# arkworks-rs/poly-commit

Hardware: AMD Instinct MI355X
Metric: MSM G1-scalar-pairs/sec inside KZG commit+open (MarlinKZG10<Bls12_381> shape, hiding off), inputs HBM-resident (host-input blocking calls: value_trait_shaped) (higher is better)
Workload: dtype u32 limbs (381-bit Fq / 255-bit Fr modular integer); 1 GPU; MarlinKZG10<bls12_381> commit+open, dense poly deg 2^24 per GPU, true SRS resident, hiding off (BASELINE metric sizes: 2^20 = configs[1], 2^24 = north-star target); curve=bls12_381, log_degree=24, inflight=2, srs_window_table=True, parallelism=1 GPU

## Files before the change

### poly_commit_amd/csrc/ec.hpp

```cpp
#pragma once
#include "fp32.hpp"
#include "fp30.hpp"
#include "fp2.hpp"

namespace pc {

template <class C1> struct G2Of { typedef C1 Base; typedef typename C1::FqP FqP; typedef typename C1::FrP FrP; };
template <class C> struct CoordOf { typedef Fd<typename C::FqP> type; };
template <class C1> struct CoordOf<G2Of<C1>> { typedef Fq2D<typename C1::FqP> type; };
template <class C> struct ScalarCurveOf { typedef C type; static constexpr bool IS_G2 = false; };
template <class C1> struct ScalarCurveOf<G2Of<C1>> { typedef C1 type; static constexpr bool IS_G2 = true; };
#ifndef PC_TE_DERIVED_TD
#define PC_TE_DERIVED_TD 1
#endif
template <class T> struct TeOf { typedef T Curve; typedef typename T::FqP FqP; typedef typename T::FrP FrP; };
template <class T> struct CoordOf<TeOf<T>> { typedef Fd<typename T::FqP> type; };
template <class T> struct ScalarCurveOf<TeOf<T>> { typedef TeOf<T> type; static constexpr bool IS_G2 = false; };
template <class C> struct GroupKind {
  static constexpr bool IS_TE = false, TABLE_FREE = ScalarCurveOf<C>::IS_G2, MANY_MSM = !ScalarCurveOf<C>::IS_G2, TWO_LANE = !ScalarCurveOf<C>::IS_G2;
};
template <class T> struct GroupKind<TeOf<T>> { static constexpr bool IS_TE = true, TABLE_FREE = true, MANY_MSM = true, TWO_LANE = false; };

template <class C>
struct AffD {
// ... 34 lines not shown
    r.Y = M.mul_add_mul(S.sub(r.X), W.neg(), a.y);
    r.ZZ = V; r.ZZZ = W;
    return r;
  }
  PC_HD XyzzD dbl() const {
    if (is_inf() || Y.is_zero()) return infinity();
    XyzzD r;
    Fq U = Y.dbl(), V = U.sqr(), W = U.mul(V), S = X.mul(V);
    Fq xx = X.sqr(), M = xx.dbl().add(xx);
    r.X = M.sqr().sub(S.dbl());
    r.Y = M.mul_add_mul(S.sub(r.X), W.neg(), Y);
    r.ZZ = V.mul(ZZ); r.ZZZ = W.mul(ZZZ);
    return r;
  }
  PC_HD void add_affine(const AffD<C>& a) {
    if (a.is_inf()) return;
    if (is_inf()) { X = a.x; Y = a.y; ZZ = Fq::one(); ZZZ = Fq::one(); return; }
    Fq U2 = a.x.mul(ZZ), S2 = a.y.mul(ZZZ);
    Fq Pp = U2.sub(X), R = S2.sub(Y);
    if (Pp.is_zero()) {
      if (R.is_zero()) *this = dbl_affine(a); else *this = infinity();
      return;
    }
    Fq PP = Pp.sqr(), PPP = Pp.mul(PP), Q = X.mul(PP);
    Fq X3 = R.sqr().sub(PPP).sub(Q.dbl());
    Y = R.mul_add_mul(Q.sub(X3), Y.neg(), PPP);
    X = X3;
    ZZ = ZZ.mul(PP); ZZZ = ZZZ.mul(PPP);
  }
  PC_HD void add_affine_lz(const AffD<C>& a, bool negate) {
    if (a.y.is_zero()) { if (a.x.is_zero()) return; }
    const Fq ay = negate ? a.y.neg_lz_canonical() : a.y;
    if (is_inf()) { X = a.x; Y = ay; ZZ = Fq::one(); ZZZ = Fq::one(); return; }
    Fq U2 = a.x.mul_lz(ZZ), S2 = ay.mul_lz(ZZZ);
    Fq Pp = U2.sub_lz(X), R = S2.sub_lz(Y);
    if (Pp.is_zero_lz()) {
      XyzzD t = canonical();
      AffD<C> b; b.x = a.x; b.y = ay.canon();
      t.add_affine(b);
      *this = t;
      return;
    }
    Fq PP = Pp.sqr_lz(), PPP = Pp.mul_lz(PP), Q = X.mul_lz(PP);
    Fq X3 = R.sqr_lz().sub_lz(PPP).sub_lz(Q.dbl_lz());
    Y = R.mul_add_mul_lz(Q.sub_lz(X3), Y.neg_lz(), PPP);
    X = X3;
    ZZ = ZZ.mul_lz(PP); ZZZ = ZZZ.mul_lz(PPP);
  }
  PC_HD XyzzD canonical() const { XyzzD r; r.X = X.canon1(); r.Y = Y.canon1(); r.ZZ = ZZ.canon1(); r.ZZZ = ZZZ.canon1(); return r; }
  PC_HD void add(const XyzzD& o) {
    if (o.is_inf()) return;
    if (is_inf()) { *this = o; return; }
    Fq U1 = X.mul(o.ZZ), U2 = o.X.mul(ZZ), S1 = Y.mul(o.ZZZ), S2 = o.Y.mul(ZZZ);
    Fq Pp = U2.sub(U1), R = S2.sub(S1);
    if (Pp.is_zero()) {
      if (R.is_zero()) *this = dbl(); else *this = infinity();
      return;
    }
    Fq PP = Pp.sqr(), PPP = Pp.mul(PP), Q = U1.mul(PP);
    Fq X3 = R.sqr().sub(PPP).sub(Q.dbl());
    Y = R.mul_add_mul(Q.sub(X3), S1.neg(), PPP);
    X = X3;
    ZZ = ZZ.mul(o.ZZ).mul(PP); ZZZ = ZZZ.mul(o.ZZZ).mul(PPP);
  }
  PC_HD AffD<C> to_affine() const {
    if (is_inf()) return AffD<C>::infinity();
    Fq t = ZZ.mul(ZZZ).inv();
    AffD<C> a; a.x = X.mul(t.mul(ZZZ)); a.y = Y.mul(t.mul(ZZ)); return a;
  }
};


struct XyzzR30 {
  typedef pc_curve_bls12_381 C;
  typedef Fd<C::FqP> F32;
  typedef Fq30 Fq;
  Fq X, Y, ZZ, ZZZ;

  static PC_HD XyzzR30 infinity() { XyzzR30 r; r.X = Fq::zero(); r.Y = Fq::zero(); r.ZZ = Fq::zero(); r.ZZZ = Fq::zero(); return r; }
  PC_HD bool is_inf() const { return ZZ.is_zero_exact(); }
  PC_HD XyzzD<C> to32() const { XyzzD<C> r; r.X = X.to32(); r.Y = Y.to32(); r.ZZ = ZZ.to32(); r.ZZZ = ZZZ.to32(); return r; }
  static PC_HD XyzzR30 from32(const XyzzD<C>& p) {
    XyzzR30 r; r.X = Fq::from32(p.X); r.Y = Fq::from32(p.Y); r.ZZ = Fq::from32(p.ZZ).reduce(); r.ZZZ = Fq::from32(p.ZZZ).reduce(); return r;
  }
  PC_HD void add_affine(const AffD<C>& a, bool negate) {
    if (a.y.is_zero()) { if (a.x.is_zero()) return; }
    const F32 ay32 = negate ? a.y.neg_lz_canonical() : a.y;
    const Fq ax = Fq::from32(a.x), ay = Fq::from32(ay32);
    if (is_inf()) { X = ax; Y = ay; ZZ = Fq::one(); ZZZ = Fq::one(); return; }
    const Fq U2 = Fq::mul<64, 2>(ax, ZZ), S2 = Fq::mul<64, 2>(ay, ZZZ);
    const Fq Pp = Fq::sub<64>(U2, X), R = Fq::sub<64>(S2, Y);
    if (Pp.is_zero_modp<66>()) {
      if (R.is_zero_modp<66>()) { AffD<C> b; b.x = a.x; b.y = ay32.canon(); *this = from32(XyzzD<C>::dbl_affine(b)); }
      else *this = infinity();
      return;
    }
    const Fq PP = Fq::sqr<66>(Pp);
    const Fq PPP = Fq::mul<66, 8>(Pp, PP), Q = Fq::mul<64, 8>(X, PP);
    const Fq RR = Fq::sqr<66>(R);
    const Fq X3 = Fq::sub_dbl<4>(Fq::sub<2>(RR, PPP), Q);
    const Fq T = Fq::sub<14>(Q, X3), NY = Fq::neg<64>(Y);
    Y = Fq::mul_add_mul<66, 16, 64, 2>(R, T, NY, PPP);
    X = X3;
    ZZ = Fq::mul<2, 8>(ZZ, PP); ZZZ = Fq::mul<2, 2>(ZZZ, PPP);
    static_assert(Fq::mul_out(64 * 2) <= 2 && Fq::mul_out(66 * 66) <= 8 && Fq::mul_out(66 * 8) <= 2 && Fq::mul_out(64 * 8) <= 2, "classes of add_affine");
    static_assert(Fq::mul_out(66 * 16 + 64 * 2) <= 64 && 8 + 2 + 4 <= 64 && Fq::mul_out(2 * 8) <= 2 && Fq::mul_out(2 * 2) <= 2, "the invariant closes");
  }
};


template <class C>
struct HalfPt {
  typedef Fd<typename C::FqP> Fq;
  Fq a, b;
  static PC_HD HalfPt of(const XyzzD<C>& p, bool odd) { HalfPt h; h.a = odd ? p.Y : p.X; h.b = odd ? p.ZZZ : p.ZZ; return h; }
};
template <class Fq>
PC_HD Fq fq_sel(bool c, const Fq& x, const Fq& y) {
  Fq r;
  PC_UNROLL for (int i = 0; i < Fq::N; i++) r.l[i] = c ? x.l[i] : y.l[i];
  return r;
}
template <class C>
struct HalfAdd {
  typedef Fd<typename C::FqP> Fq;
  Fq T1, D, DD, BB, T5, rc1, R6, X3;
  PC_HD bool p1(const HalfPt<C>& p, const HalfPt<C>& o) { T1 = p.a.mul(o.b); const Fq T2 = o.a.mul(p.b); D = T2.sub(T1); return D.is_zero(); }
  PC_HD Fq p2(const HalfPt<C>& p, const HalfPt<C>& o, bool odd) { DD = D.sqr(); BB = p.b.mul(o.b); T5 = D.mul(DD); return fq_sel(odd, DD, T5); }
  PC_HD Fq p3(bool odd, const Fq& recv) {
    rc1 = recv;
    R6 = fq_sel(odd, BB, T1).mul(fq_sel(odd, rc1, DD));
    X3 = rc1.sub(T5).sub(R6.dbl());
    return R6.sub(X3);
  }
  PC_HD void p4(HalfPt<C>& p, bool odd, const Fq& rc2) {
    const Fq R7 = fq_sel(odd, D, BB).mul_add_mul(fq_sel(odd, rc2, DD), fq_sel(odd, T1.neg(), Fq::zero()), fq_sel(odd, rc1, Fq::zero()));
    p.a = fq_sel(odd, R7, X3);
    p.b = fq_sel(odd, R6, R7);
  }
};

template <class C>
struct JacD {
  typedef Fd<typename C::FqP> Fq;
  Fq X, Y, Z;
  static PC_HD JacD infinity() { JacD r; r.X = Fq::one(); r.Y = Fq::one(); r.Z = Fq::zero(); return r; }
  PC_HD bool is_inf() const { return Z.is_zero(); }
  PC_HD JacD dbl() const {
    if (is_inf() || Y.is_zero()) return infinity();
    Fq A = X.sqr(), B = Y.sqr(), Cc = B.sqr();
    Fq t = X.add(B).sqr().sub(A).sub(Cc);
    Fq D = t.dbl(), E = A.dbl().add(A), F = E.sqr();
    JacD r;
    r.X = F.sub(D.dbl());
    r.Z = Y.mul(Z).dbl();
    r.Y = E.mul(D.sub(r.X)).sub(Cc.dbl().dbl().dbl());
    return r;
  }
  PC_HD void add_affine(const AffD<C>& a) {
    if (a.is_inf()) return;
    if (is_inf()) { X = a.x; Y = a.y; Z = Fq::one(); return; }
    Fq Z1Z1 = Z.sqr(), U2 = a.x.mul(Z1Z1), S2 = a.y.mul(Z).mul(Z1Z1);
    Fq H = U2.sub(X), rr = S2.sub(Y);
    if (H.is_zero()) {
      if (rr.is_zero()) *this = dbl(); else *this = infinity();
      return;
// ... 76 lines not shown
```

### poly_commit_amd/csrc/msm.hpp

```cpp
#pragma once
#include <stddef.h>
#include <stdint.h>
#include <algorithm>
#include <stdexcept>
#include <vector>
#include "ec.hpp"
#include "glv.hpp"
#include "host_tail.hpp"

#if defined(__HIP_DEVICE_COMPILE__)
#define PC_ARRIVED(PT, IDX)                                                                                             \
  do {                                                                                                                  \
    constexpr int PC_N_ = sizeof((PT).x.l) / 4;                                                                         \
    for (int pc_i_ = 0; pc_i_ < PC_N_; pc_i_ += 4) asm volatile("" ::"v"((PT).x.l[pc_i_]), "v"((PT).y.l[pc_i_]));     \
    asm volatile("" ::"v"(IDX));                                                                                        \
  } while (0)
#define PC_ARRIVED_WORD(W) asm volatile("" ::"v"(W))
#define PC_ARRIVED_TD(PT)                                                                                               \
  do {                                                                                                                  \
    constexpr int PC_N_ = sizeof((PT).td.l) / 4;                                                                        \
    for (int pc_i_ = 0; pc_i_ < PC_N_; pc_i_ += 4) asm volatile("" ::"v"((PT).td.l[pc_i_]));                          \
  } while (0)
#define PC_ARRIVED_FQ2(PT, IDX)                                                                                         \
  do {                                                                                                                  \
// ... 146 lines not shown
    PC_UNROLL for (int h = 0; h < 2; h++) {
      PC_UNROLL for (int k = 0; k < 4; k++) o[5 * h + k] = hv.m[h][k];
      o[5 * h + 4] = hv.m[h][4] | (hv.neg[h] << 31);
    }
  }
};
template <class C, class Geo, class F>
PC_HD void for_each_signed_digit(const Geo& g, const uint32_t* scalar, F f) {
  if constexpr (HasGlv<C>::value) { if (g.glv) { for_each_signed_digit_t<C, 1>(g, scalar, f); return; } }
  for_each_signed_digit_t<C, 0>(g, scalar, f);
}

template <class C>
struct DigitsHistBody {
  typedef typename C::FrP FrP;
  MsmGeom g;
  const uint32_t* scalars;
  uint32_t* hist;
  PC_HD void operator()(uint32_t i) const {
    uint32_t sub, j; g.split(i, sub, j);
    for_each_signed_digit<C>(g, g.scalar_at(scalars, i, sub, j, FrP::N), [&](uint32_t h, uint32_t w, uint32_t mag, uint32_t) {
      atomic_inc_u32(hist + (size_t)g.key_window(w, sub, h) * g.nb_win + (mag - 1));
    });
  }
};

template <class C>
struct ScatterBody {
  typedef typename C::FrP FrP;
  MsmGeom g;
  const uint32_t* scalars;
  uint32_t* cursor;
  uint32_t* entries;
  PC_HD void operator()(uint32_t i) const {
    uint32_t sub, j; g.split(i, sub, j);
    for_each_signed_digit<C>(g, g.scalar_at(scalars, i, sub, j, FrP::N), [&](uint32_t h, uint32_t w, uint32_t mag, uint32_t neg) {
      const uint32_t pos = atomic_inc_u32(cursor + (size_t)g.key_window(w, sub, h) * g.nb_win + (mag - 1));
      entries[pos] = g.base_index(w, j) | (neg << 31);
    });
  }
};

PC_HD uint32_t find_bucket(const uint32_t* offs, uint32_t nb, uint32_t v) {
  uint32_t lo = 0, hi = nb;
  while (hi - lo > 1) {
    uint32_t mid = (lo + hi) >> 1;
    if (offs[mid] <= v) lo = mid; else hi = mid;
  }
  return lo;
}

PC_HD void partial_slot_range(const uint32_t* offs, uint32_t key, uint32_t T, uint32_t T2, uint32_t T2b, uint32_t level,
                              uint32_t& lo, uint32_t& hi) {
  lo = 2 * (offs[key] / T);
  hi = 2 * ((offs[key + 1] - 1) / T);
  for (uint32_t l = 2; l <= level; l++) { const uint32_t d = (l == 2) ? T2 : T2b; lo = 2 * (lo / d); hi = 2 * (hi / d); }
}

template <class C> struct AccSum { static constexpr bool R30 = false; typedef XyzzD<C> type; };
#if PC_ACC_R30
template <> struct AccSum<pc_curve_bls12_381> { static constexpr bool R30 = true; typedef XyzzR30 type; };
#endif
PC_HD constexpr uint32_t acc_stage_word(uint32_t tid, uint32_t piece, uint32_t pieces) { return ((tid >> 6) * pieces + piece) * 256u + (tid & 63u) * 4u; }
template <class C>
struct StageRegs {
  AffD<C> nxt;
  PC_HD void gather(const uint32_t* src) { nxt = AffD<C>::load(src); }
  PC_HD AffD<C> take() const { return nxt; }
  PC_HD void done() const {}
};
template <class C>
struct AccumulateBody {
  typedef XyzzD<C> Pt;
  typedef typename AccSum<C>::type Sum;
  static constexpr bool R30 = AccSum<C>::R30;
  static constexpr int AW = AffD<C>::WORDS;
  MsmGeom g;
  const uint32_t* bases;
  const uint32_t* entries;
  const uint32_t* offsets;
  uint32_t* buckets;
  uint32_t* pkeys;
  uint32_t* ppts;
  static constexpr bool LAZY = Pt::Fq::LAZY_OK;
  static constexpr bool LAZY_STORE = LAZY && Pt::Fq::LAZY_STORE_OK;
  static PC_HD Pt store_form(const Pt& acc) { if constexpr (LAZY && !LAZY_STORE) return acc.canonical(); else return acc; }
  static PC_HD Pt store_form(const XyzzR30& acc) { static_assert(!R30 || LAZY_STORE, "to32() hands over lazily reduced coordinates"); return acc.to32(); }
  PC_HD void flush(const Pt& acc_lz, uint32_t k, bool complete, uint32_t t, bool first, uint32_t& k0, uint32_t& k1) const {
    const Pt& acc = acc_lz;
    if (complete) { acc.store(buckets + (size_t)k * Pt::WORDS); return; }
    uint32_t slot = first ? 2 * t : 2 * t + 1;
    acc.store(ppts + (size_t)slot * Pt::WORDS);
    if (first) k0 = k; else k1 = k;
  }
  template <class Stage = StageRegs<C>>
  PC_HD void chunk(uint32_t t, uint32_t& k0, uint32_t& k1, Pt& last, Stage st = Stage()) const {
    const uint32_t M = offsets[g.NB];
    const uint64_t s64 = (uint64_t)t * g.T;
    k0 = KEY_INVALID; k1 = KEY_INVALID;
    if (s64 < M) {
      const uint32_t s = (uint32_t)s64;
      const uint32_t e = (M - s > g.T) ? s + g.T : M;
      uint32_t k = find_bucket(offsets, g.NB, s);
      uint32_t run_lo = offsets[k], boundary = offsets[k + 1];
      uint32_t next_boundary = offsets[k + 2 <= g.NB ? k + 2 : g.NB];
      Sum acc = Sum::infinity();
      bool first = true;
      uint32_t val = entries[s];
      uint32_t nval = (s + 1 < e) ? entries[s + 1] : val;
      constexpr bool PREFETCH_PT = !ScalarCurveOf<C>::IS_G2;
      AffD<C> pt = AffD<C>::load(bases + (size_t)(val & PC_ACC_DEBUG_IDX_MASK) * g.pt_stride);
      for (uint32_t p = s; p < e; p++) {
        if constexpr (ScalarCurveOf<C>::IS_G2) PC_ARRIVED_FQ2(pt, nval); else PC_ARRIVED(pt, nval);
#if PC_TE_DERIVED_TD
        if constexpr (GroupKind<C>::IS_TE) PC_ARRIVED_TD(pt);
#endif
        PC_ARRIVED_WORD(next_boundary);
        if (p == boundary) {
          flush(store_form(acc), k, run_lo >= s, t, first, k0, k1);
          first = false; acc = Sum::infinity();
          k++; run_lo = p; boundary = next_boundary;
          while (boundary <= p) { k++; boundary = offsets[k + 1]; }
        }
        if constexpr (PREFETCH_PT) {
        st.gather(bases + (size_t)(nval & PC_ACC_DEBUG_IDX_MASK) * g.pt_stride);
        const uint32_t nnval = entries[p + 2 < e ? p + 2 : e - 1];
        next_boundary = offsets[k + 2 <= g.NB ? k + 2 : g.NB];
        if constexpr (R30) acc.add_affine(pt, (val >> 31) != 0);
        else if constexpr (LAZY) acc.add_affine_lz(pt, (val >> 31) != 0); else acc.add_affine(pt.neg_if(val >> 31));
        val = nval; nval = nnval; pt = st.take();
        } else {
          const uint32_t nnval = entries[p + 2 < e ? p + 2 : e - 1];
          next_boundary = offsets[k + 2 <= g.NB ? k + 2 : g.NB];
          acc.add_affine(pt.neg_if(val >> 31));
          val = nval; nval = nnval;
          pt = AffD<C>::load(bases + (size_t)(val & PC_ACC_DEBUG_IDX_MASK) * g.pt_stride);
        }
      }
      st.done();
      if constexpr (R30) {
        last = store_form(acc);
        flush(last, k, run_lo >= s && boundary <= e, t, first, k0, k1);
      } else {
        acc = store_form(acc);
        flush(acc, k, run_lo >= s && boundary <= e, t, first, k0, k1);
        last = acc;
      }
    }
  }
  PC_HD void operator()(uint32_t t) const {
    uint32_t k0, k1; Pt last;
    chunk(t, k0, k1, last);
    pkeys[2 * t] = k0; pkeys[2 * t + 1] = k1;
  }
};

template <class C>
struct SegReduceBody {
  static constexpr bool LATENCY_BOUND = true;
  typedef XyzzD<C> Pt;
  MsmGeom g;
  uint32_t level;
  uint32_t n_in;
  const uint32_t* in_keys; const uint32_t* in_pts;
  const uint32_t* offsets;
  uint32_t* buckets;
  uint32_t* out_keys; uint32_t* out_pts;
  PC_HD void flush(const Pt& acc, uint32_t key, uint32_t cs, uint32_t ce, uint32_t u, bool first, uint32_t& k0, uint32_t& k1) const {
    uint32_t lo, hi; partial_slot_range(offsets, key, g.T, g.T2, g.T2b, level, lo, hi);
    if (lo >= cs && hi < ce) { acc.store(buckets + (size_t)key * Pt::WORDS); return; }
    uint32_t slot = first ? 2 * u : 2 * u + 1;
    acc.store(out_pts + (size_t)slot * Pt::WORDS);
    if (first) k0 = key; else k1 = key;
  }
  PC_HD void operator()(uint32_t u) const {
    const uint32_t T2l = level == 1 ? g.T2 : g.T2b;
    const uint32_t cs = u * T2l;
    const uint32_t ce = (n_in - cs > T2l) ? cs + T2l : n_in;
    uint32_t k0 = KEY_INVALID, k1 = KEY_INVALID;
    uint32_t cur = KEY_INVALID; bool first = true;
    Pt acc = Pt::infinity();
    for (uint32_t p = cs; p < ce; p++) {
      uint32_t key = in_keys[p];
      if (key == KEY_INVALID) continue;
      if (key != cur) {
        if (cur != KEY_INVALID) { flush(acc, cur, cs, ce, u, first, k0, k1); first = false; }
        cur = key; acc = Pt::infinity();
      }
      acc.add(Pt::load(in_pts + (size_t)p * Pt::WORDS));
    }
    if (cur != KEY_INVALID) flush(acc, cur, cs, ce, u, first, k0, k1);
    out_keys[2 * u] = k0; out_keys[2 * u + 1] = k1;
  }
};

template <class C>
struct BucketLevelBody {
  static constexpr bool LATENCY_BOUND = true;
  typedef XyzzD<C> Pt;
  uint32_t K, weight_off, cnt, n_old;
  const uint32_t* x;
  const uint32_t* old_in;
  uint32_t* out;
  PC_HD void operator()(uint32_t lane) const {
    const uint32_t a = lane / cnt, gidx = lane % cnt;
    const size_t stride = (size_t)cnt * Pt::WORDS;
    if (a == 0) {
      const uint32_t* base = x + (size_t)gidx * K * Pt::WORDS;
      Pt run = Pt::infinity(), acc = Pt::infinity();
      if constexpr (ScalarCurveOf<C>::IS_G2) {
        for (uint32_t j = K; j-- > 0;) {
          run.add(Pt::load(base + (size_t)j * Pt::WORDS));
          if (j + weight_off > 0) acc.add(run);
        }
      } else {
      Pt nxt = Pt::load(base + (size_t)(K - 1) * Pt::WORDS);
      for (uint32_t j = K; j-- > 0;) {
        const Pt cur = nxt;
        nxt = Pt::load(base + (size_t)(j > 0 ? j - 1 : 0) * Pt::WORDS);
        run.add(cur);
        if (j + weight_off > 0) acc.add(run);
      }
      }
      run.store(out + (size_t)gidx * Pt::WORDS);
      acc.store(out + stride + (size_t)gidx * Pt::WORDS);
    } else {
      const uint32_t* base = old_in + (size_t)(a - 1) * cnt * K * Pt::WORDS + (size_t)gidx * K * Pt::WORDS;
      Pt acc = Pt::infinity();
      if constexpr (ScalarCurveOf<C>::IS_G2) {
        for (uint32_t j = 0; j < K; j++) acc.add(Pt::load(base + (size_t)j * Pt::WORDS));
      } else {
      Pt nxt = Pt::load(base);
      for (uint32_t j = 0; j < K; j++) {
        const Pt cur = nxt;
        nxt = Pt::load(base + (size_t)(j + 1 < K ? j + 1 : j) * Pt::WORDS);
        acc.add(cur);
// ... 273 lines not shown
inline MsmLevels msm_plan_levels(const MsmConfig& cfg, const MsmGeom& g, size_t n, bool tbl) {
  MsmLevels lv;
  uint32_t m = g.nb_win;
  uint32_t kbits = 0;
  while (m > 1) {
    uint32_t K;
    const size_t level_pts = (size_t)n * g.Wd <= cfg.coop2_max_entries ? (size_t)g.W * m * (1 + (lv.n_levels ? lv.narr[lv.n_levels - 1] : 0))
                                                                         : (size_t)-1;
    if ((size_t)g.W * m > cfg.coop_max_points) K = tbl ? cfg.tbl_K0 : cfg.K0;
    else {
      uint32_t rem = 0; while ((1u << rem) < m) rem++;
      uint32_t lg1 = 0; while ((1u << lg1) < cfg.K1) lg1++;
      if (level_pts <= cfg.coop2_max_points && lg1 > 7) lg1 = 7;
      const uint32_t nl = (rem + lg1 - 1) / lg1;
      K = 1u << ((rem + nl - 1) / nl);
    }
    if (K > m) K = m;
    uint32_t lgK = 0; while ((1u << lgK) < K) lgK++;
    const bool bits = K >= 16;
    const uint32_t woff = lv.n_levels == 0 ? 1u : 0u;
    const uint32_t nw = bits ? lgK + woff : 1u;
    lv.K[lv.n_levels] = K; m /= K; lv.m[lv.n_levels] = m;
    lv.mode[lv.n_levels] = !bits ? 0u : (K <= 128 && level_pts <= cfg.coop2_max_points) ? 2u : 1u;
    lv.narr[lv.n_levels] = nw + (lv.n_levels ? lv.narr[lv.n_levels - 1] : 0);
    std::vector<uint32_t> e;
    if (bits) { for (uint32_t b = 0; b < lgK; b++) e.push_back(kbits + b); if (woff) e.push_back(kbits); }
    else e.push_back(kbits);
    e.insert(e.end(), lv.arr_exp.begin(), lv.arr_exp.end());
    lv.arr_exp.swap(e);
    kbits += lgK;
    lv.n_levels++;
  }
  return lv;
}

template <class C, class Backend>
class MsmPlan {
 public:
  typedef XyzzD<C> Pt;
  typedef typename C::FrP FrP;
  typedef typename ScalarCurveOf<C>::type SC;
  static constexpr bool G2 = GroupKind<C>::TABLE_FREE;
  static constexpr int AW = AffD<C>::WORDS;

  MsmPlan(Backend& be, size_t n_max, const MsmConfig& cfg, uint32_t subs = 0) : be_(be), cfg_(cfg), n_max_(n_max), subs_(subs) {
    if (subs_ && (!cfg_.tbl || !cfg_.tbl_c || n_max % subs_)) throw std::runtime_error("MsmPlan: many-MSM mode needs a window table");
    if (G2 && (subs_ ? !GroupKind<C>::MANY_MSM : cfg_.tbl != nullptr)) throw std::runtime_error("MsmPlan: G2 and twisted Edwards groups are table-free");
    if (cfg_.T2 < 4) cfg_.T2 = 4;
    if (cfg_.T2b < 4) cfg_.T2b = 4;
    auto pow2_floor = [](uint32_t v, uint32_t lo, uint32_t hi) { uint32_t p = lo; while (p * 2 <= v && p * 2 <= hi) p *= 2; return p; };
    cfg_.K0 = pow2_floor(cfg_.K0, 2, 1u << 12);
    cfg_.tbl_K0 = pow2_floor(cfg_.tbl_K0, 2, 1u << 12);
    cfg_.K1 = pow2_floor(cfg_.K1, 2, 256);
    if (cfg_.T2 > 4096) cfg_.T2 = 4096;
    if (cfg_.T2b > 4096) cfg_.T2b = 4096;
    min_T_ = cfg_.T ? cfg_.T : 16;
    size_t NBmax = 1, Mmax = 1, red_max = 1, res_max = 1;
    std::vector<size_t> sizes;
    if (subs_) sizes.push_back(n_max);
    else {
      for (size_t p2 = 1; p2 <= n_max; p2 <<= 1) { sizes.push_back(p2); if (p2 > 1) sizes.push_back(p2 - 1); if (p2 > (n_max >> 1)) break; }
      sizes.push_back(31); sizes.push_back(32); sizes.push_back(n_max);
      if (cfg_.tbl && cfg_.tbl_min_n) { sizes.push_back(cfg_.tbl_min_n); if (cfg_.tbl_min_n > 1) sizes.push_back(cfg_.tbl_min_n - 1); }
    }
    for (size_t n : sizes) {
      if (n < 1 || n > n_max) continue;
      plan_geometry(n);
      NBmax = std::max<size_t>(NBmax, g_.NB);
      Mmax = std::max<size_t>(Mmax, n * (size_t)g_.Wd);
      size_t total = 0;
      for (uint32_t l = 0; l < n_levels_; l++) total += (size_t)(1 + lvl_narr_[l]) * g_.W * lvl_m_[l];
      red_max = std::max(red_max, total);
      res_max = std::max<size_t>(res_max, (size_t)g_.W * (n_levels_ ? lvl_narr_[n_levels_ - 1] : 1));
    }
    entries_cap_ = Mmax; nb_cap_ = NBmax;
    if (!cfg_.T && Mmax <= ((size_t)1 << 17)) min_T_ = 8;
    hist_ = offsets_ = cursor_ = entries_ = buckets_ = scalars_ = red_ = nullptr; pk_[0] = pk_[1] = pp_[0] = pp_[1] = nullptr;
    try {
    hist_ = (uint32_t*)be_.alloc((NBmax + 1) * 4);
    offsets_ = (uint32_t*)be_.alloc((NBmax + 1) * 4);
    cursor_ = (uint32_t*)be_.alloc((NBmax + 1) * 4);
    entries_ = (uint32_t*)be_.alloc(Mmax * 4);
    buckets_ = (uint32_t*)be_.alloc(NBmax * Pt::WORDS * 4);
    scalars_ = (uint32_t*)be_.alloc((n_max ? n_max : 1) * (size_t)FrP::N * 4);
    size_t lanes0 = ceil_div_u32(Mmax, min_T_);
    if (!cfg_.T) {
      const size_t tl = std::max(cfg_.target_lanes, cfg_.tbl ? (cfg_.tbl_chunk ? std::max(cfg_.tbl_max_lanes, cfg_.tbl_target_lanes) : cfg_.tbl_target_lanes) : 0u);
      size_t bound = std::max<size_t>(tl * 17 / 16 + 2, Mmax / 4096 + 1);
      if (lanes0 > bound) lanes0 = bound;
    }
    size_t slots = 2 * lanes0;
    part_slots_ = slots;
    for (int i = 0; i < 2; i++) {
      pk_[i] = (uint32_t*)be_.alloc(slots * 4);
      pp_[i] = (uint32_t*)be_.alloc(slots * (size_t)Pt::WORDS * 4);
      slots = 2 * (size_t)ceil_div_u32(slots, cfg_.T2);
    }
    red_ = (uint32_t*)be_.alloc((red_max + 2 * (size_t)subs_) * (size_t)Pt::WORDS * 4);
    result_host_ = (uint32_t*)be_.alloc_host(std::max<size_t>(res_max, 2 * (size_t)subs_) * Pt::WORDS * 4);
    red_points_ = red_max;
    } catch (...) { release(); throw; }
    plan_geometry(n_max);
  }
  ~MsmPlan() { release(); }
  void release() {
    void* ps[] = {hist_, offsets_, cursor_, entries_, buckets_, scalars_, pk_[0], pk_[1], pp_[0], pp_[1], red_, entries2_, offsets2_, buckets2_, hist2_, cursor2_};
    entries2_ = offsets2_ = buckets2_ = hist2_ = cursor2_ = nullptr;
    for (void* p : ps) be_.free(p);
    be_.free_host(result_host_);
    be_.free(tab_); be_.free_host(tab_host_); tab_ = nullptr; tab_host_ = nullptr;
    hist_ = offsets_ = cursor_ = entries_ = buckets_ = scalars_ = red_ = nullptr; pk_[0] = pk_[1] = pp_[0] = pp_[1] = nullptr;
    result_host_ = nullptr;
  }

  void trim() {
    if (in_parts_) return;
    void* ps[] = {entries2_, offsets2_, buckets2_, hist2_, cursor2_};
    entries2_ = offsets2_ = buckets2_ = hist2_ = cursor2_ = nullptr;
    for (void* p : ps) be_.free(p);
  }

  const MsmGeom& geom() const { return g_; }
  uint32_t* scalar_staging() { return scalars_; }
  const MsmGeom& last_geom() const { return g_; }

  void run(const uint32_t* bases_dev, uint32_t base_off, const uint32_t* scalars_dev, size_t n, bool from_mont,
           uint32_t* out_host) {
    enqueue(bases_dev, base_off, scalars_dev, n, from_mont);
    finish(out_host);
  }

  void enqueue_vectors(const uint32_t* bases_dev, uint32_t base_off, const uint64_t* ptrs_host, size_t count, size_t m, bool from_mont) {
    if (!subs_ || count > subs_ || count * m > n_max_) throw MsmCapacityError("MsmPlan: batch exceeds the plan");
    if (!tab_) { tab_ = (uint64_t*)be_.alloc((size_t)subs_ * 8); tab_host_ = (uint64_t*)be_.alloc_host((size_t)subs_ * 8); }
    for (size_t k = 0; k < count; k++) tab_host_[k] = ptrs_host[k];
    be_.copy_h2d(tab_, tab_host_, count * 8);
    enqueue(bases_dev, base_off, nullptr, count * m, from_mont, m, tab_);
  }

  void enqueue(const uint32_t* bases_dev, uint32_t base_off, const uint32_t* scalars_dev, size_t n, bool from_mont,
               size_t m_sub = 0, const uint64_t* scalar_tab = nullptr) {
    pending_empty_ = (n == 0);
    if (n == 0) return;
    plan_geometry(n);
    parts_k_ = 0; in_parts_ = false;
    part_body(bases_dev, base_off, scalars_dev, n, from_mont, m_sub, scalar_tab, true, true);
    reduce_and_download();
  }

  void begin_parts(size_t n_total) {
    if (subs_) throw std::runtime_error("MsmPlan: parts are for single MSMs");
    pending_empty_ = (n_total == 0);
    if (n_total == 0) return;
    if (n_total > n_max_) throw MsmCapacityError("MsmPlan: call exceeds the workspace this plan was sized for");
    plan_geometry(n_total);
    parts_k_ = 0; in_parts_ = true; parts_n_ = 0;
    if (!entries2_) {
      entries2_ = (uint32_t*)be_.alloc(entries_cap_ * 4);
      offsets2_ = (uint32_t*)be_.alloc((nb_cap_ + 1) * 4);
      buckets2_ = (uint32_t*)be_.alloc(nb_cap_ * Pt::WORDS * 4);
      hist2_ = (uint32_t*)be_.alloc((nb_cap_ + 1) * 4);
      cursor2_ = (uint32_t*)be_.alloc((nb_cap_ + 1) * 4);
    }
    set_tok_[0] = set_tok_[1] = -1;
  }
  void add_part(const uint32_t* bases_dev, uint32_t base_off, const uint32_t* scalars_dev, size_t n, bool from_mont, int ready_tok, bool last) {
    if (pending_empty_ || n == 0) { if (last && !pending_empty_) { if (parts_k_ == 0) { pending_empty_ = true; return; } reduce_and_download(); } return; }
    part_body(bases_dev, base_off, scalars_dev, n, from_mont, 0, nullptr, parts_k_ == 0, last, ready_tok);
    parts_n_ += n;
    if (last) reduce_and_download();
  }

 private:
  void part_body(const uint32_t* bases_dev, uint32_t base_off, const uint32_t* scalars_dev, size_t n, bool from_mont, size_t m_sub,
                 const uint64_t* scalar_tab, bool first, bool last, int ready_tok = -1) {
    MsmGeom g = g_;
    g.n = (uint32_t)n; g.base_off = base_off; g.from_mont = from_mont ? 1 : 0;
    g.m_sub = subs_ ? (uint32_t)(m_sub ? m_sub : n / subs_) : 0u;
    g.scalar_tab = scalar_tab;
    const size_t Mmax = n * g.Wd;
    uint32_t want_lanes = g.tbl_stride ? cfg_.tbl_target_lanes : cfg_.target_lanes;
    if (g.tbl_stride && cfg_.tbl_chunk)
      while ((uint64_t)want_lanes * 2 <= cfg_.tbl_max_lanes && Mmax / ((size_t)want_lanes * 2) >= cfg_.tbl_chunk) want_lanes *= 2;
    uint32_t T = cfg_.T ? cfg_.T : (uint32_t)((Mmax + want_lanes - 1) / want_lanes);
    if (T < min_T_) T = min_T_;
    if (T > 4096) T = 4096;
    g.T = T; g.T2 = cfg_.T2; g.T2b = cfg_.T2b;
    const size_t lanes = ceil_div_u32(Mmax, T);
    if (n > n_max_ || Mmax > entries_cap_ || g.NB > nb_cap_ || 2 * lanes > part_slots_)
      throw MsmCapacityError("MsmPlan: call exceeds the workspace this plan was sized for");
    const int set = in_parts_ ? (int)(parts_k_ & 1u) : 0;
    uint32_t* entries = set ? entries2_ : entries_; uint32_t* offsets = set ? offsets2_ : offsets_;
    uint32_t* hist = set ? hist2_ : hist_; uint32_t* cursor = set ? cursor2_ : cursor_;
    uint32_t* buckets = (in_parts_ && !first) ? buckets2_ : buckets_;
    const bool marks = !in_parts_ || first;
    be_.memset(buckets, 0, (size_t)g.NB * Pt::WORDS * 4);
    if (in_parts_) {
      int tok = -1;
      {
        struct AuxScope { Backend& b; bool marks_was; int* tok; ~AuxScope() { b.timing_marks(marks_was); try { *tok = b.aux_end(); } catch (...) { *tok = -1; } } };
        be_.aux_begin(set_tok_[set], ready_tok);
        AuxScope scope{be_, be_.timing_marks(marks), &tok};
        be_.template sort_entries<SC>(g, scalars_dev, hist, offsets, cursor, entries);
      }
      be_.wait_token(tok);
    } else {
      be_.template sort_entries<SC>(g, scalars_dev, hist, offsets, cursor, entries);
    }

    { AccumulateBody<C> b{g, g.tbl_stride ? cfg_.tbl : bases_dev, entries, offsets, buckets, pk_[0], pp_[0]}; be_.template accumulate<C>(b, lanes); }
    if (!in_parts_ || last) be_.mark();
    const bool tail_queue = !in_parts_ && n <= ((size_t)3 << 19);
    struct TailGuard { Backend& b; bool armed; ~TailGuard() { if (armed) b.end_tail(); } } tail_guard{be_, false};
    if (tail_queue) { be_.begin_tail(); tail_guard.armed = true; }
    size_t slots = 2 * lanes; uint32_t level = 1; int cur = 0;
    for (;;) {
      size_t lanes2 = ceil_div_u32(slots, level == 1 ? g.T2 : g.T2b);
      if (lanes2 <= (cfg_.seg_tail_lanes ? cfg_.seg_tail_lanes : 1u)) {
        be_.template seg_reduce_tail<C>(g, level, (uint32_t)slots, pk_, pp_, cur, offsets, buckets);
        break;
      }
      SegReduceBody<C> b{g, level, (uint32_t)slots, pk_[cur], pp_[cur], offsets, buckets, pk_[cur ^ 1], pp_[cur ^ 1]};
      be_.launch(b, lanes2);
      slots = 2 * lanes2; level++; cur ^= 1;
    }
    if (in_parts_) {
      if (!first) { BucketMergeBody<C> m{buckets_, buckets2_}; be_.launch(m, g.NB); }
      set_tok_[set] = be_.main_token();
      parts_k_++;
    }
    last_g_ = g;
    tail_open_ = tail_queue; tail_guard.armed = false;
  }

  void reduce_and_download() {
    const MsmGeom& g = last_g_;
    struct TailScope { Backend& b; bool on; ~TailScope() { if (on) b.end_tail(); } } tail_scope{be_, tail_open_};
    tail_open_ = false;
    be_.mark();
    const uint32_t* x = buckets_;
    uint32_t* lvl_base = red_;
    uint32_t* prev_base = nullptr;
    for (uint32_t l = 0; l < n_levels_; l++) {
      const uint32_t K = lvl_K_[l], m_out = lvl_m_[l];
      const size_t cnt = (size_t)g.W * m_out;
      const size_t stride = cnt * Pt::WORDS;
      const uint32_t n_old = l ? lvl_narr_[l - 1] : 0;
      const uint32_t* old_in = l ? prev_base + (size_t)g.W * lvl_m_[l - 1] * Pt::WORDS : nullptr;
      be_.template bucket_level<C>(K, l == 0 ? 1u : 0u, (uint32_t)cnt, n_old, (int)lvl_bits_[l], x, old_in, lvl_base);
      x = lvl_base; prev_base = lvl_base; lvl_base += (size_t)(1 + lvl_narr_[l]) * stride;
    }
    be_.mark();
    if (subs_) {
      SubFoldBody<C> f;
      f.arrays = n_levels_ ? prev_base + (size_t)g.W * Pt::WORDS : buckets_;
      f.W = g.W; f.narr = n_levels_ ? (uint32_t)arr_exp_.size() : 1u;
      if (f.narr > 32) throw std::runtime_error("MsmPlan: too many reduction arrays");
      for (uint32_t a = 0; a < f.narr; a++) { f.exp[a] = n_levels_ ? arr_exp_[a] : 0u; f.order[a] = a; }
      std::stable_sort(f.order, f.order + f.narr, [&](uint32_t x, uint32_t y) { return f.exp[x] > f.exp[y]; });
      f.out = red_ + red_points_ * Pt::WORDS;
      be_.launch(f, g.W);
      be_.copy_d2h_async(result_host_, f.out, (size_t)g.W * Pt::WORDS * 4);
    }
    else if (n_levels_ == 0) be_.copy_d2h_async(result_host_, buckets_, (size_t)g.W * Pt::WORDS * 4);
    else be_.copy_d2h_async(result_host_, prev_base + (size_t)g.W * Pt::WORDS, (size_t)g.W * lvl_narr_[n_levels_ - 1] * Pt::WORDS * 4);
    be_.record_done();
    in_parts_ = false;
  }

 public:
  void prepare_replay(size_t n) { pending_empty_ = (n == 0); if (n) plan_geometry(n); }

  void finish(uint32_t* out_host) {
    if (subs_) {
      if constexpr (GroupKind<C>::IS_TE) {
        if (pending_empty_) { std::vector<uint32_t> empty((size_t)subs_ * Pt::WORDS, 0u); host64::batch_to_affine<C>(empty.data(), subs_, out_host); return; }
        be_.wait_done();
        host64::batch_to_affine<C>(result_host_, subs_, out_host);
        return;
      }
      if (pending_empty_) { for (size_t i = 0; i < (size_t)subs_ * AW; i++) out_host[i] = 0; return; }
      be_.wait_done();
      if constexpr (!G2) if (g_.glv) {
        typedef host64::Xyzz64<C> P64;
        std::vector<uint32_t> sum((size_t)subs_ * Pt::WORDS);
        for (uint32_t k = 0; k < subs_; k++) {
          P64 a = P64::load(result_host_ + (size_t)(2 * k) * Pt::WORDS), b = P64::load(result_host_ + (size_t)(2 * k + 1) * Pt::WORDS);
          b.X = b.X.mul(P64::Fq::load(GlvOf<C>::T::BETA_MONT));
          a.add(b);
          a.store(&sum[(size_t)k * Pt::WORDS]);
        }
        host64::batch_to_affine<C>(sum.data(), subs_, out_host);
        return;
      }
      host64::batch_to_affine<C>(result_host_, subs_, out_host);
      return;
    }
    if (pending_empty_) { for (int i = 0; i < AW; i++) out_host[i] = 0; return; }
    if (in_parts_) {
      be_.quiesce();
      in_parts_ = false; tail_open_ = false;
      throw std::runtime_error("MsmPlan: a call in parts was abandoned before its last part");
    }
    be_.wait_done();
    host_tail(out_host);
  }

 private:
  void plan_geometry(size_t n) {
    const bool tbl = subs_ || (cfg_.tbl && cfg_.tbl_c && n >= cfg_.tbl_min_n);
    uint32_t c = tbl ? cfg_.tbl_c : cfg_.c ? cfg_.c : msm_choose_c(n, FrP::BITS);
    g_ = msm_make_geom(FrP::BITS, n, c, tbl, tbl && cfg_.tbl_glv, subs_, cfg_.tbl_stride, tbl ? cfg_.tbl_pt_stride : (uint32_t)AW, cfg_.T2, cfg_.T2b);
    const MsmLevels lv = msm_plan_levels(cfg_, g_, n, tbl);
    n_levels_ = lv.n_levels;
    for (uint32_t l = 0; l < lv.n_levels; l++) { lvl_K_[l] = lv.K[l]; lvl_m_[l] = lv.m[l]; lvl_bits_[l] = lv.mode[l]; lvl_narr_[l] = lv.narr[l]; }
    arr_exp_ = lv.arr_exp;
  }

  void host_tail(uint32_t* out_host) {
    const uint32_t L = n_levels_, W = g_.W;
    const uint32_t cw = g_.tbl_stride ? 0u : g_.c;
    const size_t narr = L == 0 ? 1 : arr_exp_.size();
    if constexpr (!G2) if (g_.glv) {
      typedef host64::Xyzz64<C> P64;
      for (size_t a = 0; a < narr; a++) {
        uint32_t* p = &result_host_[(a * W + 1) * Pt::WORDS];
        P64::Fq::load(p).mul(P64::Fq::load(GlvOf<C>::T::BETA_MONT)).store(p);
      }
    }
    std::vector<host64::WeightedPoint> items;
    if (L == 0) {
      for (uint32_t w = 0; w < W; w++) items.push_back({cw * w, &result_host_[(size_t)w * Pt::WORDS]});
    } else {
      for (size_t a = 0; a < arr_exp_.size(); a++)
        for (uint32_t w = 0; w < W; w++)
          items.push_back({cw * w + arr_exp_[a], &result_host_[(a * W + w) * Pt::WORDS]});
    }
    host64::horner_to_affine<C>(items, out_host);
  }

  Backend& be_;
  MsmConfig cfg_;
  size_t n_max_;
  uint32_t subs_ = 0;
  size_t red_points_ = 0;
  MsmGeom g_;
  uint32_t min_T_;
  size_t part_slots_ = 0, entries_cap_ = 0, nb_cap_ = 0;
  uint32_t *hist_, *offsets_, *cursor_, *entries_, *buckets_, *scalars_, *red_;
  uint32_t* pk_[2]; uint32_t* pp_[2];
  uint32_t n_levels_; uint32_t lvl_K_[32]; uint32_t lvl_m_[32]; uint32_t lvl_bits_[32]; uint32_t lvl_narr_[32];
  std::vector<uint32_t> arr_exp_;
  uint32_t* result_host_ = nullptr;
  uint64_t* tab_ = nullptr; uint64_t* tab_host_ = nullptr;
  bool pending_empty_ = true;
  uint32_t *entries2_ = nullptr, *offsets2_ = nullptr, *buckets2_ = nullptr, *hist2_ = nullptr, *cursor2_ = nullptr;
  uint32_t parts_k_ = 0; size_t parts_n_ = 0; bool in_parts_ = false, tail_open_ = false;
  int set_tok_[2] = {-1, -1};
  MsmGeom last_g_;
};

}
```

### poly_commit_amd/csrc/msm_coop.hpp

```cpp
#pragma once
#include <hip/hip_runtime.h>
#include "msm.hpp"

namespace pc {

template <class C>
struct LdsPoints {
  typedef XyzzD<C> Pt;
  uint32_t* base; uint32_t lanes;
  __device__ __forceinline__ void put(uint32_t lane, const Pt& p) const {
    uint32_t w[Pt::WORDS]; p.store(w);
#pragma unroll
    for (int k = 0; k < Pt::WORDS; k++) base[k * lanes + lane] = w[k];
  }
  __device__ __forceinline__ Pt get(uint32_t lane) const {
    uint32_t w[Pt::WORDS];
#pragma unroll
    for (int k = 0; k < Pt::WORDS; k++) w[k] = base[k * lanes + lane];
    return Pt::load(w);
  }
};

template <class C>
__global__ void __launch_bounds__(256) k_bucket_level_coop(uint32_t K, uint32_t lgK, uint32_t weight_off, uint32_t cnt, uint32_t n_old,
// ... 79 lines not shown
    for (int k = 0; k < FN; k++) { smem[k * L + tid] = v.a.l[k]; smem[(FN + k) * L + tid] = v.b.l[k]; }
  };
  auto get = [&](uint32_t t2) {
    HalfPt<C> r;
#pragma unroll
    for (int k = 0; k < FN; k++) { r.a.l[k] = smem[k * L + t2]; r.b.l[k] = smem[(FN + k) * L + t2]; }
    return r;
  };
  auto store = [&](uint32_t* dst) { v.a.store(dst + oa); v.b.store(dst + ob); };
  if (a == 0) {
    for (uint32_t d = 0; d < lgK; d++) {
      put();
      __syncthreads();
      const uint32_t low = l & ((2u << d) - 1u);
      if ((low & (low - 1u)) == 0 && low < (1u << d)) half_add<C>(v, get(tid + (2u << d)), odd);
      __syncthreads();
    }
    uint32_t* o = out + (size_t)gidx * Pt::WORDS;
    if (l == 0) { store(o); if (weight_off) store(o + (size_t)(1 + lgK) * stride); }
    else if ((l & (l - 1u)) == 0) { uint32_t b = 31 - __builtin_clz(l); store(o + (size_t)(1 + b) * stride); }
  } else {
    for (uint32_t d = K >> 1; d >= 1; d >>= 1) {
      put();
      __syncthreads();
      if (l < d) half_add<C>(v, get(tid + 2 * d), odd);
      __syncthreads();
    }
    if (l == 0) store(out + (size_t)(nw + a) * stride + (size_t)gidx * Pt::WORDS);
  }
}

#ifndef PC_ACC_WAVES_PER_EU
#define PC_ACC_WAVES_PER_EU 1
#endif
#ifndef PC_ACC_WAVES_N8
#define PC_ACC_WAVES_N8 1
#endif
#ifndef PC_ACC_LDS_STAGE
#define PC_ACC_LDS_STAGE 1
#endif
template <class C> struct AccStage { static constexpr bool LDS = PC_ACC_LDS_STAGE && AccSum<C>::R30 && !ScalarCurveOf<C>::IS_G2; };
template <class C>
struct StageLds {
  typedef __attribute__((address_space(3))) uint32_t lds_u32;
  typedef uint32_t u32x4 __attribute__((ext_vector_type(4)));
  typedef __attribute__((address_space(3))) u32x4 lds_u128;
  static constexpr uint32_t PIECES = AffD<C>::WORDS / 4;
  lds_u32* tile; uint32_t tid;
  __device__ __forceinline__ void gather(const uint32_t* src) const {
    const uint32_t wave = __builtin_amdgcn_readfirstlane(tid >> 6);
#pragma unroll
    for (uint32_t j = 0; j < PIECES; j++)
      __builtin_amdgcn_global_load_lds((const __attribute__((address_space(1))) void*)(src + 4 * j),
                                       (__attribute__((address_space(3))) void*)(tile + acc_stage_word(wave << 6, j, PIECES)), 16, 0, 0);
  }
  __device__ __forceinline__ AffD<C> take() const {
    uint32_t w[AffD<C>::WORDS];
#pragma unroll
    for (uint32_t j = 0; j < PIECES; j++) {
      const u32x4 v = *(const lds_u128*)(tile + acc_stage_word(tid, j, PIECES));
      w[4 * j] = v.x; w[4 * j + 1] = v.y; w[4 * j + 2] = v.z; w[4 * j + 3] = v.w;
    }
    return AffD<C>::load(w);
  }
  __device__ __forceinline__ void done() const { asm volatile("s_waitcnt vmcnt(0)" ::: "memory"); }
};
template <class C> struct AccTune {
  static constexpr int WAVES = Fd<typename C::FqP>::N <= 8 ? PC_ACC_WAVES_N8 : (AccSum<C>::R30 && PC_ACC_WAVES_PER_EU < 2) ? 2 : PC_ACC_WAVES_PER_EU;
  static constexpr uint32_t WG = ScalarCurveOf<C>::IS_G2 ? 128u : 256u;
};
#define PC_ACC_BOUNDS __launch_bounds__(AccTune<C>::WG, AccTune<C>::WAVES)
template <class C>
__global__ void PC_ACC_BOUNDS k_accumulate(AccumulateBody<C> b, uint32_t lanes) {
  typedef XyzzD<C> Pt;
  constexpr uint32_t WG = AccTune<C>::WG;
  __shared__ __attribute__((aligned(AccStage<C>::LDS ? 16 : 4))) uint32_t xch[Pt::WORDS * WG];
  __shared__ uint32_t key_out[WG], key_first[WG], flags[WG];
  const uint32_t tid = threadIdx.x, t = blockIdx.x * WG + tid;
  const bool valid = t < lanes;
  uint32_t k0 = KEY_INVALID, k1 = KEY_INVALID;
  Pt V = Pt::infinity();
  if constexpr (AccStage<C>::LDS) {
    static_assert(AffD<C>::WORDS * WG <= Pt::WORDS * WG && WG % 64 == 0, "the stage lies inside the exchange tile");
    if (valid) b.chunk(t, k0, k1, V, StageLds<C>{(typename StageLds<C>::lds_u32*)xch, tid});
  } else {
  if (valid) b.chunk(t, k0, k1, V);
  }
  const uint32_t M = b.offsets[b.g.NB];
  const uint64_t s64 = (uint64_t)t * b.g.T;
  const uint32_t cs = s64 < M ? (uint32_t)s64 : M;
  const uint32_t ce = (M - cs > b.g.T) ? cs + b.g.T : M;
  const bool head_left = k0 != KEY_INVALID && b.offsets[k0] < cs;
  const bool head_right = k0 != KEY_INVALID && k1 == KEY_INVALID && b.offsets[k0 + 1] > ce;
  const bool transparent = head_left && head_right;
  const uint32_t okey = k1 != KEY_INVALID ? k1 : head_right ? k0 : KEY_INVALID;
  LdsPoints<C> lds{xch, WG};
  uint32_t fl = (okey == KEY_INVALID || !transparent) ? 1u : 0u;
  for (uint32_t d = 1; d < WG; d <<= 1) {
    const bool need = !(fl & 1u);
    if (!__syncthreads_or(need)) break;
    if (okey != KEY_INVALID) lds.put(tid, V);
    flags[tid] = fl;
    __syncthreads();
    if (need) {
      if (tid < d) fl = 3u;
      else { V.add(lds.get(tid - d)); fl = flags[tid - d]; }
    }
    __syncthreads();
  }
  key_out[tid] = okey; key_first[tid] = head_left ? k0 : KEY_INVALID; flags[tid] = fl;
  if (okey != KEY_INVALID) lds.put(tid, V);
  __syncthreads();
  const bool take = head_left && tid > 0 && key_out[tid - 1] == k0;
  const bool give = okey != KEY_INVALID && tid < WG - 1 && key_first[tid + 1] == okey;
  if (transparent) {
    if (give) k0 = KEY_INVALID;
    else V.store(b.ppts + (size_t)(2 * t) * Pt::WORDS);
  } else {
    if (take) {
      uint32_t* slot = b.ppts + (size_t)(2 * t) * Pt::WORDS;
      Pt f = Pt::load(slot);
      f.add(lds.get(tid - 1));
      if (!(flags[tid - 1] & 2u) && !head_right) { f.store(b.buckets + (size_t)k0 * Pt::WORDS); k0 = KEY_INVALID; }
      else f.store(slot);
    }
    if (give) { if (k1 != KEY_INVALID) k1 = KEY_INVALID; else k0 = KEY_INVALID; }
  }
  if (valid) { b.pkeys[2 * t] = k0; b.pkeys[2 * t + 1] = k1; }
}

static constexpr uint32_t EDGE_REACH = 8;
template <class C>
__global__ void __launch_bounds__(64) k_accumulate_edges(AccumulateBody<C> b, uint32_t lanes) {
  PC_LATENCY_KERNEL();
  typedef XyzzD<C> Pt;
  constexpr uint32_t WG = AccTune<C>::WG;
  const uint32_t k = blockIdx.x * 64 + threadIdx.x;
  const uint64_t t64 = (uint64_t)(k + 1) * WG;
  if (t64 >= lanes) return;
  const uint32_t t = (uint32_t)t64, a = t - 1;
  const uint32_t M = b.offsets[b.g.NB];
  uint32_t aslot = 2 * a + 1, key = b.pkeys[aslot];
  if (key == KEY_INVALID) {
    aslot = 2 * a; key = b.pkeys[aslot];
    if (key == KEY_INVALID || (uint64_t)b.offsets[key + 1] <= t64 * b.g.T) return;
  }
  uint32_t u = t;
  for (;; u++) {
    if (u >= lanes || u - t >= EDGE_REACH) return;
    const uint32_t ku = b.pkeys[2 * u];
    if (ku == key) break;
    if (ku != KEY_INVALID) return;
  }
  const uint64_t us = (uint64_t)u * b.g.T;
  const uint32_t ue = (M - (uint32_t)us > b.g.T) ? (uint32_t)us + b.g.T : M;
  uint32_t* slot = b.ppts + (size_t)(2 * u) * Pt::WORDS;
  Pt f = Pt::load(slot);
  f.add(Pt::load(b.ppts + (size_t)aslot * Pt::WORDS));
  b.pkeys[aslot] = KEY_INVALID;
  const uint64_t ws = (uint64_t)(a - (WG - 1u)) * b.g.T;
  if (b.offsets[key] >= ws && b.offsets[key + 1] <= ue) { f.store(b.buckets + (size_t)key * Pt::WORDS); b.pkeys[2 * u] = KEY_INVALID; }
  else f.store(slot);
}

template <class C>
__global__ void __launch_bounds__(256) k_seg_reduce_tail(MsmGeom g, uint32_t level, uint32_t slots, uint32_t* pk0, uint32_t* pk1,
                                                         uint32_t* pp0, uint32_t* pp1, int cur, const uint32_t* offsets,
                                                         uint32_t* buckets) {
  PC_LATENCY_KERNEL();
// ... 15 lines not shown
```

Measured before the change: 545.9 million pairs/s.

## Store radix-2^30 bucket sums raw and convert to 32-bit form in a separate pass

Within the accumulate loop, bucket flushes now write the radix-2^30 XYZZ accumulator in its raw limb layout with 128-bit vector stores, skipping the per-flush to32 conversion. Complete buckets go to a new raw buffer and are converted by a follow-up kernel over all buckets. The lane's first partial run is converted in place after the loop. The intent is to take the conversion arithmetic and its register pressure out of the hot accumulation loop. The cost is an extra kernel launch, an extra buffer, and more memory traffic. The LDS-stage path forces RAW=true, which relies on the static_assert that the sum is R30.

```diff
diff --git a/poly_commit_amd/csrc/ec.hpp b/poly_commit_amd/csrc/ec.hpp
--- a/poly_commit_amd/csrc/ec.hpp
+++ b/poly_commit_amd/csrc/ec.hpp
@@ -140,6 +140,29 @@
   PC_HD XyzzD<C> to32() const { XyzzD<C> r; r.X = X.to32(); r.Y = Y.to32(); r.ZZ = ZZ.to32(); r.ZZZ = ZZZ.to32(); return r; }
   static PC_HD XyzzR30 from32(const XyzzD<C>& p) {
     XyzzR30 r; r.X = Fq::from32(p.X); r.Y = Fq::from32(p.Y); r.ZZ = Fq::from32(p.ZZ).reduce(); r.ZZZ = Fq::from32(p.ZZZ).reduce(); return r;
+  }
+  static constexpr int RAW_WORDS = 4 * Fq::N;
+  PC_HD void store_raw(uint32_t* o) const {
+    uint32_t w[RAW_WORDS];
+    PC_UNROLL for (int i = 0; i < Fq::N; i++) { w[i] = X.l[i]; w[Fq::N + i] = Y.l[i]; w[2 * Fq::N + i] = ZZ.l[i]; w[3 * Fq::N + i] = ZZZ.l[i]; }
+#if defined(__HIP_DEVICE_COMPILE__)
+    typedef uint32_t u32x4 __attribute__((ext_vector_type(4)));
+    PC_UNROLL for (int j = 0; j < RAW_WORDS / 4; j++) { u32x4 v; v.x = w[4 * j]; v.y = w[4 * j + 1]; v.z = w[4 * j + 2]; v.w = w[4 * j + 3]; ((u32x4*)o)[j] = v; }
+#else
+    for (int i = 0; i < RAW_WORDS; i++) o[i] = w[i];
+#endif
+  }
+  static PC_HD XyzzR30 load_raw(const uint32_t* p) {
+    uint32_t w[RAW_WORDS];
+#if defined(__HIP_DEVICE_COMPILE__)
+    typedef uint32_t u32x4 __attribute__((ext_vector_type(4)));
+    PC_UNROLL for (int j = 0; j < RAW_WORDS / 4; j++) { const u32x4 v = ((const u32x4*)p)[j]; w[4 * j] = v.x; w[4 * j + 1] = v.y; w[4 * j + 2] = v.z; w[4 * j + 3] = v.w; }
+#else
+    for (int i = 0; i < RAW_WORDS; i++) w[i] = p[i];
+#endif
+    XyzzR30 r;
+    PC_UNROLL for (int i = 0; i < Fq::N; i++) { r.X.l[i] = w[i]; r.Y.l[i] = w[Fq::N + i]; r.ZZ.l[i] = w[2 * Fq::N + i]; r.ZZZ.l[i] = w[3 * Fq::N + i]; }
+    return r;
   }
   PC_HD void add_affine(const AffD<C>& a, bool negate) {
     if (a.y.is_zero()) { if (a.x.is_zero()) return; }
diff --git a/poly_commit_amd/csrc/msm.hpp b/poly_commit_amd/csrc/msm.hpp
--- a/poly_commit_amd/csrc/msm.hpp
+++ b/poly_commit_amd/csrc/msm.hpp
@@ -252,6 +252,7 @@
   uint32_t* buckets;
   uint32_t* pkeys;
   uint32_t* ppts;
+  uint32_t* buckets_raw;
   static constexpr bool LAZY = Pt::Fq::LAZY_OK;
   static constexpr bool LAZY_STORE = LAZY && Pt::Fq::LAZY_STORE_OK;
   static PC_HD Pt store_form(const Pt& acc) { if constexpr (LAZY && !LAZY_STORE) return acc.canonical(); else return acc; }
@@ -263,8 +264,9 @@
     acc.store(ppts + (size_t)slot * Pt::WORDS);
     if (first) k0 = k; else k1 = k;
   }
-  template <class Stage = StageRegs<C>>
+  template <class Stage = StageRegs<C>, bool RAW = false>
   PC_HD void chunk(uint32_t t, uint32_t& k0, uint32_t& k1, Pt& last, Stage st = Stage()) const {
+    static_assert(!RAW || R30, "only the radix-2^30 sum has a raw form");
     const uint32_t M = offsets[g.NB];
     const uint64_t s64 = (uint64_t)t * g.T;
     k0 = KEY_INVALID; k1 = KEY_INVALID;
@@ -287,6 +289,12 @@
 #endif
         PC_ARRIVED_WORD(next_boundary);
         if (p == boundary) {
+          if constexpr (RAW) {
+            static_assert(!RAW || Sum::RAW_WORDS <= 2 * Pt::WORDS, "the raw first run lies inside the lane's two partial slots");
+            const bool complete = run_lo >= s;
+            acc.store_raw(complete ? buckets_raw + (size_t)k * Sum::RAW_WORDS : ppts + (size_t)(2 * t) * Pt::WORDS);
+            if (!complete) k0 = k;
+          } else
           flush(store_form(acc), k, run_lo >= s, t, first, k0, k1);
           first = false; acc = Sum::infinity();
           k++; run_lo = p; boundary = next_boundary;
@@ -308,6 +316,9 @@
         }
       }
       st.done();
+      if constexpr (RAW) {
+        if (k0 != KEY_INVALID) { uint32_t* slot = ppts + (size_t)(2 * t) * Pt::WORDS; Sum::load_raw(slot).to32().store(slot); }
+      }
       if constexpr (R30) {
         last = store_form(acc);
         flush(last, k, run_lo >= s && boundary <= e, t, first, k0, k1);
@@ -320,8 +331,21 @@
   }
   PC_HD void operator()(uint32_t t) const {
     uint32_t k0, k1; Pt last;
-    chunk(t, k0, k1, last);
+    this->template chunk<StageRegs<C>, R30>(t, k0, k1, last);
     pkeys[2 * t] = k0; pkeys[2 * t + 1] = k1;
+  }
+};
+
+struct BucketRawBody {
+  typedef XyzzD<pc_curve_bls12_381> Pt;
+  const uint32_t* offsets; const uint32_t* raw; uint32_t* buckets; uint32_t T, NB;
+  PC_HD void operator()(uint32_t k) const {
+    const uint32_t lo = offsets[k], hi = offsets[k + 1], M = offsets[NB];
+    if (hi == lo) return;
+    const uint64_t e64 = ((uint64_t)(lo / T) + 1) * T;
+    const uint32_t e = e64 < M ? (uint32_t)e64 : M;
+    if (hi >= e) return;
+    XyzzR30::load_raw(raw + (size_t)k * XyzzR30::RAW_WORDS).to32().store(buckets + (size_t)k * Pt::WORDS);
   }
 };
 
@@ -761,6 +785,7 @@
     cursor_ = (uint32_t*)be_.alloc((NBmax + 1) * 4);
     entries_ = (uint32_t*)be_.alloc(Mmax * 4);
     buckets_ = (uint32_t*)be_.alloc(NBmax * Pt::WORDS * 4);
+    if constexpr (AccumulateBody<C>::R30) buckets_raw_ = (uint32_t*)be_.alloc(NBmax * AccumulateBody<C>::Sum::RAW_WORDS * 4);
     scalars_ = (uint32_t*)be_.alloc((n_max ? n_max : 1) * (size_t)FrP::N * 4);
     size_t lanes0 = ceil_div_u32(Mmax, min_T_);
     if (!cfg_.T) {
@@ -783,8 +808,8 @@
   }
   ~MsmPlan() { release(); }
   void release() {
-    void* ps[] = {hist_, offsets_, cursor_, entries_, buckets_, scalars_, pk_[0], pk_[1], pp_[0], pp_[1], red_, entries2_, offsets2_, buckets2_, hist2_, cursor2_};
-    entries2_ = offsets2_ = buckets2_ = hist2_ = cursor2_ = nullptr;
+    void* ps[] = {hist_, offsets_, cursor_, entries_, buckets_, buckets_raw_, scalars_, pk_[0], pk_[1], pp_[0], pp_[1], red_, entries2_, offsets2_, buckets2_, hist2_, cursor2_};
+    entries2_ = offsets2_ = buckets2_ = hist2_ = cursor2_ = buckets_raw_ = nullptr;
     for (void* p : ps) be_.free(p);
     be_.free_host(result_host_);
     be_.free(tab_); be_.free_host(tab_host_); tab_ = nullptr; tab_host_ = nullptr;
@@ -887,7 +912,8 @@
       be_.template sort_entries<SC>(g, scalars_dev, hist, offsets, cursor, entries);
     }
 
-    { AccumulateBody<C> b{g, g.tbl_stride ? cfg_.tbl : bases_dev, entries, offsets, buckets, pk_[0], pp_[0]}; be_.template accumulate<C>(b, lanes); }
+    { AccumulateBody<C> b{g, g.tbl_stride ? cfg_.tbl : bases_dev, entries, offsets, buckets, pk_[0], pp_[0], buckets_raw_}; be_.template accumulate<C>(b, lanes); }
+    if constexpr (AccumulateBody<C>::R30) { BucketRawBody b{offsets, buckets_raw_, buckets, T, g.NB}; be_.launch(b, g.NB); }
     if (!in_parts_ || last) be_.mark();
     const bool tail_queue = !in_parts_ && n <= ((size_t)3 << 19);
     struct TailGuard { Backend& b; bool armed; ~TailGuard() { if (armed) b.end_tail(); } } tail_guard{be_, false};
@@ -1027,6 +1053,7 @@
   uint32_t min_T_;
   size_t part_slots_ = 0, entries_cap_ = 0, nb_cap_ = 0;
   uint32_t *hist_, *offsets_, *cursor_, *entries_, *buckets_, *scalars_, *red_;
+  uint32_t* buckets_raw_ = nullptr;
   uint32_t* pk_[2]; uint32_t* pp_[2];
   uint32_t n_levels_; uint32_t lvl_K_[32]; uint32_t lvl_m_[32]; uint32_t lvl_bits_[32]; uint32_t lvl_narr_[32];
   std::vector<uint32_t> arr_exp_;
diff --git a/poly_commit_amd/csrc/msm_coop.hpp b/poly_commit_amd/csrc/msm_coop.hpp
--- a/poly_commit_amd/csrc/msm_coop.hpp
+++ b/poly_commit_amd/csrc/msm_coop.hpp
@@ -185,9 +185,9 @@
   Pt V = Pt::infinity();
   if constexpr (AccStage<C>::LDS) {
     static_assert(AffD<C>::WORDS * WG <= Pt::WORDS * WG && WG % 64 == 0, "the stage lies inside the exchange tile");
-    if (valid) b.chunk(t, k0, k1, V, StageLds<C>{(typename StageLds<C>::lds_u32*)xch, tid});
-  } else {
-  if (valid) b.chunk(t, k0, k1, V);
+    if (valid) b.template chunk<StageLds<C>, true>(t, k0, k1, V, StageLds<C>{(typename StageLds<C>::lds_u32*)xch, tid});
+  } else {
+  if (valid) b.template chunk<StageRegs<C>, AccSum<C>::R30>(t, k0, k1, V);
   }
   const uint32_t M = b.offsets[b.g.NB];
   const uint64_t s64 = (uint64_t)t * b.g.T;
```

Result: no change. 546.5 million pairs/s (median of 2 runs) (+0.1%).
